# lawmurray/BayesLogit

Hardware: NVIDIA B200
Metric: pg_draws_per_sec (higher is better)
Workload: dtype f64

## Files before the change

### bayeslogit_b200/api.py

```python
import ctypes as C

import numpy as np

from . import _lib

NA = float("nan")


def set_seed(seed):
    _lib.lib().bl_set_seed(int(seed) & 0xFFFFFFFFFFFFFFFF)


def set_device(device):
    _lib.check(_lib.lib().bl_set_device(int(device)))


def _recycle(a, num, dtype):
    a = np.asarray(a, dtype=dtype).ravel()
    if a.size != num:
        a = np.resize(a, num)
    return np.ascontiguousarray(a)


def _ptr(a):
# ... 70 lines not shown


_SEEDED = {"devroye": ("bl_rpg_devroye_seeded", np.int32), "gamma": ("bl_rpg_gamma_seeded", np.float64),
           "alt": ("bl_rpg_alt_seeded", np.float64), "sp": ("bl_rpg_sp_seeded", np.float64),
           "hybrid": ("bl_rpg_hybrid_seeded", np.float64)}
_TAPE = {k: v[0].replace("_seeded", "_tape") for k, v in _SEEDED.items()}
_TAPE["devroye_plain"] = "bl_rpg_devroye_plain_tape"


def rpg_seeded(method, shape, z, seed, call_id=0, obs0=0, trunc=200):
    fn, dt = _SEEDED[method]
    z = np.ascontiguousarray(z, dtype=np.float64)
    shape = np.ascontiguousarray(shape, dtype=dt)
    num = z.size
    x = np.zeros(num)
    args = [_ptr(x), _ptr(shape), _ptr(z), num]
    it = None
    if method == "gamma":
        args.append(int(trunc))
    if method == "sp":
        it = np.zeros(num, dtype=np.int32)
        args.append(_ptr(it))
    st = getattr(_lib.lib(), fn)(*args, int(seed), int(call_id), int(obs0))
    _lib.check(st)
    return (x, it) if method == "sp" else x


def rpg_tape(method, shape, z, tape, trunc=200, trace=True):
    fn = _TAPE[method]
    dt = np.int32 if method.startswith("devroye") else np.float64
    z = np.ascontiguousarray(z, dtype=np.float64)
    shape = np.ascontiguousarray(shape, dtype=dt)
    num = z.size
    x = np.zeros(num)
    t = _lib.Tape()
    keep = []
    for k in "ueng":
        a = tape.get(k)
        if a is None:
            setattr(t, "t" + k, None)
            setattr(t, "l" + k, 0)
        else:
            a = np.ascontiguousarray(a, dtype=np.float64)
            assert a.ndim == 2 and a.shape[0] == num
            keep.append(a)
            setattr(t, "t" + k, a.ctypes.data)
            setattr(t, "l" + k, a.shape[1])
    tr = np.zeros((num, _lib.TRACE_W), dtype=np.int32) if trace else None
    args = [_ptr(x), _ptr(shape), _ptr(z), num]
    it = None
    if method == "gamma":
        args.append(int(trunc))
    if method == "sp":
        it = np.zeros(num, dtype=np.int32)
        args.append(_ptr(it))
    st = getattr(_lib.lib(), fn)(*args, C.byref(t), _ptr(tr) if trace else None)
    _lib.check(st)
    out = [x]
    if trace:
        out.append(tr)
    if it is not None:
        out.append(it)
    return tuple(out) if len(out) > 1 else x


def pg_moments(b, z):
    b = np.ascontiguousarray(b, dtype=np.float64)
    z = np.ascontiguousarray(z, dtype=np.float64)
    m1, m2 = np.zeros(b.size), np.zeros(b.size)
    _lib.check(_lib.lib().bl_probe_pg_moments(_ptr(m1), _ptr(m2), _ptr(b), _ptr(z), b.size))
    return m1, m2


def v_eval(y):
    y = np.ascontiguousarray(y, dtype=np.float64)
    v = np.zeros(y.size)
    _lib.check(_lib.lib().bl_probe_v_eval(_ptr(v), _ptr(y), y.size))
    return v


SPECFUN = {"p_norm": 0, "log_p_norm": 1, "p_gamma_rate": 2, "p_igauss": 3, "lgamma": 4, "tgamma": 5,
           "dev_right_mass": 6, "dev_coef": 7, "upper_gamma_cf": 8, "p_igauss_direct": 9, "sp_log_cos_rt": 10,
           "sp_v_table": 11, "sp_pl": 12, "sp_pl_estimate": 13,
           "alt_pr": 14, "alt_pr_estimate": 15}


def specfun(which, a, b=None, c=None):
    a = np.ascontiguousarray(a, dtype=np.float64)
    b = a if b is None else np.ascontiguousarray(np.broadcast_to(b, a.shape), dtype=np.float64)
    c = a if c is None else np.ascontiguousarray(np.broadcast_to(c, a.shape), dtype=np.float64)
    out = np.zeros(a.size)
    _lib.check(_lib.lib().bl_probe_specfun(_ptr(out), SPECFUN[which], _ptr(a), _ptr(b), _ptr(c), a.size))
    return out


def philox4x32_10(ctr, key):
    ctr = np.ascontiguousarray(ctr, dtype=np.uint32)
    key = np.ascontiguousarray(key, dtype=np.uint32)
    out = np.zeros(4, dtype=np.uint32)
    _lib.check(_lib.lib().bl_probe_philox(_ptr(out), _ptr(ctr), _ptr(key)))
    return out
```

### bayeslogit_b200/csrc/pg_alt.cuh

```cuda
#pragma once

namespace bl {

template <class Src>
__device__ __forceinline__ double alt_rtinvchi2(Src &s, double h, double trunc)
{
    double h2 = h * h;
    double R = trunc / h2;
    double E1 = s.expon();
    double E2 = s.expon();
    while ((E1 * E1) > (2 * E2 / R)) {
        E1 = s.expon();
        E2 = s.expon();
    }
    double X = 1 + E1 * R;
    X = R / (X * X);
    return h2 * X;
}

__device__ __forceinline__ double alt_pigauss(double x, double z, double lambda)
{
    double sq = sqrt(lambda / x);
    double b = sq * (x * z - 1);
    double a = sq * (x * z + 1) * -1.0;
    return p_norm(b) + ool::exp_(2 * lambda * z) * p_norm(a);
}

enum AltField {
    kAltH = 0,
    kAltTrunc,
    kAltPr,
    kAltCoef,
    kAltLgh,
    kAltLd0, kAltLd1,
    kAltLtB, kAltLtC0, kAltLtLM,
    kAltPrBand,
    kAltSetupDoubles
};
constexpr int kAltStateDoubles = 2 * kAltSetupDoubles;

struct AltState {
    double f[kAltStateDoubles];
    __device__ __forceinline__ double get(int k) const { return f[k]; }
};

struct AltStateRef {
    const double *o;
    size_t stride;
    __device__ __forceinline__ double get(int k) const { return o[(size_t)k * stride]; }
};

__device__ __forceinline__ void alt_plan(double h, int &nfull, int &nrem, double &hrem)
{
    double n = floor((h - 1.0) / 4.0);
    double remain = h - 4.0 * n;
    nfull = (int)n;
    if (remain > 4.0) {
        nrem = 2;
        hrem = 0.5 * remain;
    } else {
        nrem = 1;
        hrem = remain;
    }
}

static __device__ __noinline__ double alt_pr_fp64(double h, double z, double trunc)
{
    const double kLog2 = 0.693147180559945309417232;
    double wl, wr;
    if (z != 0)
        wl = ool::exp_(h * (kLog2 - z)) * alt_pigauss(trunc, z / h, h * h);
    else
        wl = ool::exp_(h * kLog2) * (1.0 - p_gamma_rate(1 / trunc, 0.5, 0.5 * h * h));
    double lambda_z = kPi * kPi * 0.125 + 0.5 * z * z;
    wr = ool::exp_(h * ool::log_((0.5 * kPi) / lambda_z)) * (1.0 - p_gamma_rate(trunc, h, lambda_z));
    return wr / (wr + wl);
}

constexpr double kAltPrBandWidth = 2e-5;

__device__ __forceinline__ float alt_pr_estimate(double h, double z, double trunc)
{
    const float hf = (float)h, zf = (float)z, tf = (float)trunc;
    if (!(zf < 12.0f)) return -1.0f;
    const float s = hf * rsqrtf(tf);
    const float tz = tf * zf / hf;
    const float b = s * (tz - 1.0f), na = s * (tz + 1.0f);
    const float phib = 0.5f * erfcf(-b * 0.70710678f);
    const float wl = exp2f(hf) * (__expf(-hf * zf) * phib
                                  + 0.5f * erfcxf(na * 0.70710678f) * __expf(hf * zf - 0.5f * na * na));
    const float lam = 1.2337005501361697f + 0.5f * zf * zf;
    const float x = tf * lam;
    const float lpre = hf * __logf(x) - x;
    float Q;
    if (x < hf + 1.0f) {
        float term = 1.0f, sum = 1.0f, ap = hf;
        for (int k = 0; k < 60; ++k) {
            ap += 1.0f;
            term *= x / ap;
            sum += term;
            if (term < 1e-8f * sum) break;
        }
        Q = 1.0f - sum * __expf(lpre - lgammaf(hf + 1.0f));
    } else {
        float cf = upper_gamma_cf_f32(hf, x);
        if (!(cf > 0.0f)) return -1.0f;
        Q = cf * __expf(lpre - lgammaf(hf));
    }
    if (!(Q > 0.0f)) return -1.0f;
    const float wr = __expf(hf * __logf(1.5707963267948966f / lam)) * Q;
    const float pr = wr / (wr + wl);
    return pr >= 0.0f && pr <= 1.0f ? pr : -1.0f;
}

template <bool kEstimatePr>
static __device__ __noinline__ void alt_setup(double h, double z, double *out)
{
    const double kLog2 = 0.693147180559945309417232;
    int idx = (int)floor((h - 1.0) * 100.0);
    double trunc = PG_TRUNC_SCHEDULE[idx];
    double rate_z = 0.125 * kPi * kPi + 0.5 * z * z;
    float est = kEstimatePr ? alt_pr_estimate(h, z, trunc) : -1.0f;
    out[kAltH] = h;
    out[kAltTrunc] = trunc;
    out[kAltPr] = est >= 0.0f ? (double)est : alt_pr_fp64(h, z, trunc);
    out[kAltPrBand] = est >= 0.0f ? kAltPrBandWidth : 0.0;
    out[kAltCoef] = ool::exp_(h * kLog2 - 0.5 * 1.8378770664093454835606594728112 );
    out[kAltLgh] = ool::lgamma_(h);
    out[kAltLd0] = ool::log_(h);
    out[kAltLd1] = ool::log_(2.0 + h);
    double b = rate_z * trunc;
    double d1 = b - h;
    double d3 = h - 1.0;
    double c0 = 0.5 * (d1 + sqrt(d1 * d1 + 4.0 * b)) / b;
    out[kAltLtB] = b;
    out[kAltLtC0] = c0;
    out[kAltLtLM] = d3 * ool::log_(d3 / (1.0 - c0)) - d3;
}

template <class St>
__device__ __forceinline__ bool alt_pick_right(double u, const St &st, int o, double z)
{
    const double pr = st.get(o + kAltPr), band = st.get(o + kAltPrBand);
    if (u < pr - band) return true;
    if (u > pr + band || band == 0.0) return false;
    return u < alt_pr_fp64(st.get(o + kAltH), z, st.get(o + kAltTrunc));
}

struct AltLane {
    double X, alpha, sum;
    int trial;
    int phase;
    int nfull;
    int nrem;
    __device__ __forceinline__ void start(int nf, int nr)
    {
        X = 0.0; alpha = 0.0; sum = 0.0; trial = 0; phase = 0; nfull = nf; nrem = nr;
    }
};

__device__ __forceinline__ double alt_coef(double n, double lx3, double ldn, double x, double h,
                                           double coef_h, double &g)
{
    double d_n = 2.0 * n + h;
    if (n != 0)
        g *= (n + h - 1) / n;
    else
        g = 1.0;
    double coef = coef_h * g;
    double log_kernel = -0.5 * (lx3 + d_n * d_n / x) + ldn;
    return coef * ool::exp_(log_kernel);
}

template <class Src, class St>
__device__ __forceinline__ bool alt_pick(Src &src, AltLane &L, double z, const St &st)
{
    const int o = L.nfull > 0 ? 0 : kAltSetupDoubles;
    if (L.trial >= 10000) {
        L.sum += -1.0;
        L.trial = 0;
        if (L.nfull > 0)
            L.nfull--;
        else
            L.nrem--;
        return L.nfull == 0 && L.nrem == 0;
    }
    L.trial++;
    if (alt_pick_right(src.unif(), st, o, z)) {
        L.phase = 1;
    } else {
        L.phase = (st.get(o + kAltH) / z > st.get(o + kAltTrunc)) ? 2 : 3;
        L.alpha = 0.0;
    }
    return false;
}

template <class St>
static __device__ __noinline__ bool alt_series_exact(double X, double u, double h, double trunc, const St &st, int o)
{
    const int max_inner = 200;
    const double coef_h = st.get(o + kAltCoef);
    const double lx3 = ool::log_(X * X * X);
    double g = 1.0;
    double S = alt_coef(0.0, lx3, st.get(o + kAltLd0), X, h, coef_h, g);
    double a_n = S;
    double gt;
    if (X > trunc)
        gt = ool::exp_(h * 0.45158270528945486472619522989488  + (h - 1) * (lx3 * (1.0 / 3.0))
                       - kPi * kPi * 0.125 * X - st.get(o + kAltLgh));
    else
        gt = h * ool::exp_(h * 0.693147180559945309417232 - 0.5 * (1.8378770664093454835606594728112 + lx3)
                           - 0.5 * h * h / X);
    double Y = u * gt;
    int n = 0;
    bool go = true, accept = false;
    while (go && n < max_inner) {
        ++n;
        double prev = a_n;
        double ldn = n == 1 ? st.get(o + kAltLd1) : ool::log_(2.0 * n + h);
        a_n = alt_coef((double)n, lx3, ldn, X, h, coef_h, g);
// ... 123 lines not shown
```

### bayeslogit_b200/csrc/pg_hybrid.cu

```cuda
#include <algorithm>
#include <cstdlib>
#include <vector>

#include "engine.h"
#include "pg_devroye_fast.cuh"
#include "pg_stream.cuh"

namespace bl {

namespace {

constexpr int kBinThreads = 256;
constexpr int kMetaCounts = 0;
constexpr int kMetaOffsets = 8;
constexpr int kMetaCursor = 16;

__global__ void __launch_bounds__(kBinThreads)
k_hyb_count(const double *__restrict__ h, int n, int *__restrict__ meta)
{
    __shared__ int cnt[8];
    if (threadIdx.x < 8) cnt[threadIdx.x] = 0;
    __syncthreads();
    int local[6] = {0, 0, 0, 0, 0, 0};
    for (int i = blockIdx.x * blockDim.x + threadIdx.x; i < n; i += gridDim.x * blockDim.x)
// ... 27 lines not shown
    constexpr int kCells = kBinPer * (kBinThreads / 32);
    __shared__ int wcnt[kCells][8];
    __shared__ int base[8];
    const int lane = threadIdx.x & 31, warp = threadIdx.x >> 5;
    const unsigned lt = (1u << lane) - 1u;
    const int tile_obs = kBinThreads * kBinPer;
    int tiles = (n + tile_obs - 1) / tile_obs;
    for (int tile = blockIdx.x; tile < tiles; tile += gridDim.x) {
        int reg[kBinPer], rank[kBinPer];
#pragma unroll
        for (int k = 0; k < kBinPer; ++k) {
            int i = tile * tile_obs + k * kBinThreads + threadIdx.x;
            reg[k] = i < n ? regime_of(h[i]) : -1;
        }
#pragma unroll
        for (int k = 0; k < kBinPer; ++k) {
            int i = tile * tile_obs + k * kBinThreads + threadIdx.x;
            if (reg[k] == kRegZero) x[i] = 0.0;
            rank[k] = 0;
#pragma unroll
            for (int r = 1; r < 6; ++r) {
                unsigned m = __ballot_sync(0xffffffffu, reg[k] == r);
                if (reg[k] == r) rank[k] = __popc(m & lt);
                if (lane == 0) wcnt[k * (kBinThreads / 32) + warp][r] = __popc(m);
            }
        }
        __syncthreads();
        if (threadIdx.x >= 1 && threadIdx.x < 6) {
            int r = threadIdx.x, run = 0;
            for (int c = 0; c < kCells; ++c) {
                int v = wcnt[c][r];
                wcnt[c][r] = run;
                run += v;
            }
            base[r] = run ? meta[kMetaOffsets + r] + atomicAdd(&meta[kMetaCursor + r], run) : 0;
        }
        __syncthreads();
#pragma unroll
        for (int k = 0; k < kBinPer; ++k) {
            if (reg[k] > 0) {
                int i = tile * tile_obs + k * kBinThreads + threadIdx.x;
                idx[base[reg[k]] + wcnt[k * (kBinThreads / 32) + warp][reg[k]] + rank[k]] = i;
            }
        }
        __syncthreads();
    }
}

template <int R, bool kChains = false>
__global__ void __launch_bounds__(128)
k_hyb_regime(double *__restrict__ x, const double *__restrict__ h, const double *__restrict__ z,
             const int *__restrict__ idx, const int *__restrict__ meta, StreamId id)
{
    const int count = meta[kMetaCounts + R];
    const int *list = idx + meta[kMetaOffsets + R];
    for (int j = blockIdx.x * blockDim.x + threadIdx.x; j < count; j += gridDim.x * blockDim.x) {
        int i = list[j];
        PhiloxSource s;
        if (kChains) open_batch_stream(s, id, i);
        else s.open(id.seed, id.obs0 + (uint64_t)i, id.call_id);
        double b = h[i], zi = z[i], v;
        if (R == kRegNormal) {
            double m = pg_m1(b, zi);
            double var = pg_m2(b, zi) - m * m;
            v = m + sqrt(var) * s.norm();
        } else if (R == kRegSP) {
            sp_draw(s, v, b, zi);
        } else if (R == kRegDevroye) {
            v = devroye_sum_fast(s, (int)b, zi);
        } else if (R == kRegAlt) {
            v = alt_draw(s, b, zi);
        } else {
            v = gamma_sum(s, b, zi, 200);
        }
        x[i] = v;
    }
}

__global__ void __launch_bounds__(128, 8)
k_sp_setup(const double *__restrict__ h, const double *__restrict__ z, const int *__restrict__ idx,
           const int *__restrict__ meta, double *__restrict__ state, int c0, int cap)
{
    const int count = min(meta[kMetaCounts + kRegSP] - c0, cap);
    const int *list = idx + meta[kMetaOffsets + kRegSP] + c0;
    for (int j = blockIdx.x * blockDim.x + threadIdx.x; j < count; j += gridDim.x * blockDim.x) {
        int i = list[j];
        SpState s;
        sp_setup<true>(h[i], z[i], s);
#pragma unroll
        for (int k = 0; k < kSpStateDoubles; ++k) state[(size_t)k * cap + j] = s.f[k];
    }
}

constexpr int kLaneChunk = 128;

constexpr int kRgThreads = 256;

template <int F, int D, int I>
struct RgSlots {
    double f[F][kRgThreads];
    double d[D][kRgThreads];
    uint4 buf[kRgThreads];
    uint32_t blk[kRgThreads];
    int pos[kRgThreads];
    int i[I][kRgThreads];
    int obs[kRgThreads];
    int phase[kRgThreads];
    int perm[kRgThreads];
    int wcnt[kRgThreads / 32][3];
};

struct SpRegroup {
    static constexpr int F = kSpStateDoubles, D = 3, I = 1, kClasses = 2, kRegime = kRegSP;
    using Slots = RgSlots<F, D, I>;
    __device__ static void begin(Slots &S, int t, double shape, double zraw, PhiloxSource &src)
    {
        S.d[0][t] = shape;
        S.d[1][t] = 0.5 * fabs(zraw);
        S.d[2][t] = 2.0;
        S.i[0][t] = 1;
        SpStateRef st{&S.f[0][t], (size_t)kRgThreads};
        S.phase[t] = sp_pick_left(src.unif(), st, shape) ? 1 : 2;
    }
    __device__ static bool advance(Slots &S, int sl, PhiloxSource &src, double &omega)
    {
        SpLane L;
        L.X = S.d[2][sl];
        L.iter = S.i[0][sl];
        L.phase = S.phase[sl];
        const double n = S.d[0][sl];
        SpStateRef st{&S.f[0][sl], (size_t)kRgThreads};
        bool done = sp_trip_staged(src, L, n, S.d[1][sl], st);
        if (!done && L.phase == 0) {
            if (L.iter >= 200) {
                done = true;
            } else {
                L.iter++;
                L.phase = sp_pick_left(src.unif(), st, n) ? 1 : 2;
            }
        }
        if (done) {
            omega = n * 0.25 * L.X;
        } else {
            S.d[2][sl] = L.X;
            S.i[0][sl] = L.iter;
            S.phase[sl] = L.phase;
        }
        return done;
    }
};

struct AltRegroup {
    static constexpr int F = kAltStateDoubles, D = 4, I = 3, kClasses = 3, kRegime = kRegAlt;
    using Slots = RgSlots<F, D, I>;
    __device__ static void load(const Slots &S, int sl, AltLane &L)
    {
        L.X = S.d[1][sl]; L.alpha = S.d[2][sl]; L.sum = S.d[3][sl];
        L.trial = S.i[0][sl]; L.nfull = S.i[1][sl]; L.nrem = S.i[2][sl];
        L.phase = S.phase[sl];
    }
    __device__ static void store(Slots &S, int sl, const AltLane &L)
    {
        S.d[1][sl] = L.X; S.d[2][sl] = L.alpha; S.d[3][sl] = L.sum;
        S.i[0][sl] = L.trial; S.i[1][sl] = L.nfull; S.i[2][sl] = L.nrem;
        S.phase[sl] = L.phase;
    }
    __device__ static void begin(Slots &S, int t, double shape, double zraw, PhiloxSource &src)
    {
        int nfull, nrem;
        double hrem;
        alt_plan(shape, nfull, nrem, hrem);
        AltLane L;
        L.start(nfull, nrem);
// ... 332 lines not shown
```

### bayeslogit_b200/csrc/pg_kernels.cu

```cuda
#include "engine.h"
#include "pg_devroye_fast.cuh"
#include "pg_stream.cuh"

namespace bl {

namespace {

constexpr int kThreads = 128;

inline int grid_for(int64_t num, int threads, int ctas_per_sm)
{
    int64_t need = (num + threads - 1) / threads;
    int64_t cap = 148LL * ctas_per_sm;
    return (int)(need < cap ? (need > 0 ? need : 1) : cap);
}

template <int M, class Src>
__device__ __forceinline__ double draw_one(Src &s, const void *shape, const double *z, int64_t i,
                                           int trunc, int *iter, int &aux)
{
    aux = 0;
    if (M == kDevroye || M == kDevroyeLoop) {
        int n = ((const int *)shape)[i];
        return n != 0 ? devroye_sum_fast(s, n, z[i]) : 0.0;
// ... 11 lines not shown
        if (h != 0) {
            double d;
            aux = sp_draw(s, d, h, z[i]);
            if (iter) iter[i] = aux;
            return d;
        }
        return 0.0;
    } else {
        double h = ((const double *)shape)[i];
        return hybrid_draw(s, h, z[i], aux);
    }
}

template <int M, bool kChains = false>
__global__ void __launch_bounds__(kThreads)
k_rpg_philox(double *__restrict__ x, const void *__restrict__ shape, const double *__restrict__ z,
             int64_t num, int trunc, int *__restrict__ iter, StreamId id)
{
    int64_t stride = (int64_t)gridDim.x * blockDim.x;
    for (int64_t i = (int64_t)blockIdx.x * blockDim.x + threadIdx.x; i < num; i += stride) {
        PhiloxSource s;
        if (kChains) open_batch_stream(s, id, i);
        else s.open(id.seed, id.obs0 + (uint64_t)i, id.call_id);
        int aux;
        x[i] = draw_one<M>(s, shape, z, i, trunc, iter, aux);
    }
}

template <int M>
__global__ void __launch_bounds__(kThreads)
k_rpg_tape(double *__restrict__ x, const void *__restrict__ shape, const double *__restrict__ z,
           int64_t num, int trunc, int *__restrict__ iter, DevTape tp, int *__restrict__ trace)
{
    int64_t stride = (int64_t)gridDim.x * blockDim.x;
    for (int64_t i = (int64_t)blockIdx.x * blockDim.x + threadIdx.x; i < num; i += stride) {
        TapeSource s;
        s.open(tp.tu, tp.lu, tp.te, tp.le, tp.tn, tp.ln, tp.tg, tp.lg, (size_t)i);
        int aux;
        double v = draw_one<M>(s, shape, z, i, trunc, iter, aux);
        x[i] = s.exhausted() ? nan("") : v;
        if (trace) {
            int *t = trace + i * BL_TRACE_W;
            s.counts(t);
            t[4] = s.exhausted() ? 1 : 0;
            t[5] = aux;
        }
    }
}

__global__ void k_probe_moments(double *m1, double *m2, const double *b, const double *z, int64_t num)
{
    int64_t i = (int64_t)blockIdx.x * blockDim.x + threadIdx.x;
    if (i < num) {
        m1[i] = pg_m1(b[i], z[i]);
        m2[i] = pg_m2(b[i], z[i]);
    }
}

__global__ void k_probe_v_eval(double *v, const double *y, int64_t num)
{
    int64_t i = (int64_t)blockIdx.x * blockDim.x + threadIdx.x;
    if (i < num) v[i] = v_eval(y[i]);
}

__global__ void k_probe_specfun(double *out, int which, const double *a, const double *b,
                                const double *c, int64_t num)
{
    int64_t i = (int64_t)blockIdx.x * blockDim.x + threadIdx.x;
    if (i >= num) return;
    double r = 0.0;
    switch (which) {
    case 0: r = p_norm(a[i]); break;
    case 1: r = log_p_norm(a[i]); break;
    case 2: r = p_gamma_rate(a[i], b[i], c[i]); break;
    case 3: r = p_igauss(a[i], b[i], c[i]); break;
    case 4: r = lgamma(a[i]); break;
    case 5: r = tgamma(a[i]); break;
    case 6: r = dev_right_mass(a[i]); break;
    case 7: r = dev_coef((int)b[i], a[i]); break;
    case 8: r = upper_gamma_cf(b[i], a[i]); break;
    case 9: r = p_igauss_direct(a[i], b[i], c[i]); break;
    case 10: { double v, g; sp_vg(a[i], v, g); r = g; break; }
    case 11: { double v, g; r = sp_vg_table(a[i], v, g) ? v : nan(""); break; }
    case 12: { SpState st; sp_setup<false>(a[i], b[i], st); r = st.f[kSpPl]; break; }
    case 13: { SpState st; sp_setup<true>(a[i], b[i], st); r = st.f[kSpPlBand] > 0.0 ? st.f[kSpPl] : nan(""); break; }
    case 14: { double f[kAltSetupDoubles]; alt_setup<false>(a[i], 0.5 * fabs(b[i]), f); r = f[kAltPr]; break; }
    case 15: { double f[kAltSetupDoubles]; alt_setup<true>(a[i], 0.5 * fabs(b[i]), f); r = f[kAltPrBand] > 0.0 ? f[kAltPr] : nan(""); break; }
    }
    out[i] = r;
}

__global__ void k_probe_philox(uint32_t *out4, const uint32_t *ctr4, const uint32_t *key2)
{
    uint4 r = Philox4x32::block(make_uint4(ctr4[0], ctr4[1], ctr4[2], ctr4[3]),
                                make_uint2(key2[0], key2[1]));
    out4[0] = r.x; out4[1] = r.y; out4[2] = r.z; out4[3] = r.w;
}

template <int M, bool kChains = false>
cudaError_t launch_philox_m(double *x, const void *shape, const double *z, int64_t num, int trunc,
                            int *iter, StreamId id, cudaStream_t st)
{
    if (num <= 0) return cudaSuccess;
    k_rpg_philox<M, kChains><<<grid_for(num, kThreads, 16), kThreads, 0, st>>>(x, shape, z, num, trunc, iter, id);
    count_launch();
    return cudaGetLastError();
}

template <int M>
cudaError_t launch_tape_m(double *x, const void *shape, const double *z, int64_t num, int trunc,
                          int *iter, DevTape tp, int *trace, cudaStream_t st)
{
    if (num <= 0) return cudaSuccess;
    k_rpg_tape<M><<<grid_for(num, kThreads, 16), kThreads, 0, st>>>(x, shape, z, num, trunc, iter, tp, trace);
    count_launch();
    return cudaGetLastError();
}

}

cudaError_t launch_rpg(Method m, double *x, const void *shape, const double *z, int64_t num,
                       int trunc, int *iter, StreamId id, cudaStream_t st)
{
    switch (m) {
    case kDevroye: return launch_devroye_refill(x, (const int *)shape, z, num, id, st);
    case kDevroyeLoop: return launch_philox_m<kDevroyeLoop>(x, shape, z, num, trunc, iter, id, st);
    case kGamma: return launch_philox_m<kGamma>(x, shape, z, num, trunc, iter, id, st);
    case kAlt: return launch_philox_m<kAlt>(x, shape, z, num, trunc, iter, id, st);
    case kSP: return launch_philox_m<kSP>(x, shape, z, num, trunc, iter, id, st);
    case kHybrid:
        return id.chain_len ? launch_philox_m<kHybrid, true>(x, shape, z, num, trunc, iter, id, st)
                            : launch_philox_m<kHybrid>(x, shape, z, num, trunc, iter, id, st);
    case kDevroyePlain: return launch_philox_m<kDevroyePlain>(x, shape, z, num, trunc, iter, id, st);
    }
    return cudaErrorInvalidValue;
}

cudaError_t launch_rpg_tape(Method m, double *x, const void *shape, const double *z, int64_t num,
                            int trunc, int *iter, DevTape tp, int *trace, cudaStream_t st)
{
    switch (m) {
    case kDevroye: return launch_tape_m<kDevroye>(x, shape, z, num, trunc, iter, tp, trace, st);
    case kGamma: return launch_tape_m<kGamma>(x, shape, z, num, trunc, iter, tp, trace, st);
    case kAlt: return launch_tape_m<kAlt>(x, shape, z, num, trunc, iter, tp, trace, st);
    case kSP: return launch_tape_m<kSP>(x, shape, z, num, trunc, iter, tp, trace, st);
    case kHybrid: return launch_tape_m<kHybrid>(x, shape, z, num, trunc, iter, tp, trace, st);
    case kDevroyePlain: return launch_tape_m<kDevroyePlain>(x, shape, z, num, trunc, iter, tp, trace, st);
    case kDevroyeLoop: return launch_tape_m<kDevroye>(x, shape, z, num, trunc, iter, tp, trace, st);
    }
    return cudaErrorInvalidValue;
}

cudaError_t launch_probe_moments(double *m1, double *m2, const double *b, const double *z,
                                 int64_t num, cudaStream_t st)
{
    if (num <= 0) return cudaSuccess;
    k_probe_moments<<<(unsigned)((num + 127) / 128), 128, 0, st>>>(m1, m2, b, z, num);
    count_launch();
    return cudaGetLastError();
}

cudaError_t launch_probe_v_eval(double *v, const double *y, int64_t num, cudaStream_t st)
{
    if (num <= 0) return cudaSuccess;
    k_probe_v_eval<<<(unsigned)((num + 127) / 128), 128, 0, st>>>(v, y, num);
    count_launch();
    return cudaGetLastError();
}

cudaError_t launch_probe_specfun(double *out, int which, const double *a, const double *b,
// ... 18 lines not shown
```

### bayeslogit_b200/csrc/pg_sp.cuh

```cuda
#pragma once

#include "pg_sp_tables.h"

namespace bl {

__device__ __forceinline__ double y_of_v(double v, double tol)
{
    double r = sqrt(fabs(v));
    if (v > tol) return ool::tan_(r) / r;
    if (v < -1 * tol) return ool::tanh_(r) / r;
    return 1.0;
}

static __device__ __noinline__ double v_eval_ref(double y)
{
    const double tol = 1e-9;
    const int max_iter = 1000;
    if (y < PG_YGRID[0]) return -1. / (y * y);
    if (y > PG_YGRID[PG_YGRID_LEN - 1]) {
        double v = ool::atan_(0.5 * y * kPi);
        return v * v;
    }
    if (y == 1) return 0.0;
    double id = (ool::log_(y) / ool::log_(2.0) + 4.0) / 0.1;
    int idlow = (int)id;
    int idhigh = idlow + 1;
    if (idhigh > PG_VGRID_LEN - 1) idhigh = PG_VGRID_LEN - 1;
    double vl = PG_VGRID[idlow];
    double vh = PG_VGRID[idhigh];
    int iter = 0;
    double diff = tol + 1.0;
    double vnew = vl, vold = vl;
    while (diff > tol && iter < max_iter) {
        iter++;
        vold = vnew;
        double yv = y_of_v(vold, 1e-8);
        double f0 = yv - y;
        double f1;
        if (fabs(vold) >= 1e-8)
            f1 = 0.5 * (yv * yv + (1 - yv) / vold);
        else
            f1 = 0.5 * (yv * yv);
        vnew = vold - f0 / f1;
        vnew = vnew > vh ? vh : vnew;
        vnew = vnew < vl ? vl : vnew;
        diff = fabs(vnew - vold);
    }
    return vnew;
}

__device__ __forceinline__ double sp_cos_rt(double v)
{
    double r = sqrt(fabs(v));
    return v >= 0 ? ool::cos_(r) : ool::cosh_(r);
}

__device__ __forceinline__ bool sp_vg_table(double y, double &v, double &g)
{
    if (!(y >= 0.0625 && y < 16.0)) return false;
    if (fabs(y - 1.0) < 1e-6) return false;
    float tt = (__log2f((float)y) + 4.0f) * 10.0f;
    float fr = tt - floorf(tt);
    float margin = tt > 48.0f ? 2e-4f : 5e-5f;
    if (fr < margin || fr > 1.0f - margin) return false;
    int hi = __double2hiint(y), lo = __double2loint(y);
    int e = (hi >> 20) - 1023;
    int j = (hi >> (20 - SP_TAB_K)) & ((1 << SP_TAB_K) - 1);
    double f = __hiloint2double((hi & 0x000FFFFF) | 0x3FF00000, lo);
    double u = (f - 1.0) * (double)(2 << SP_TAB_K) - (double)(2 * j + 1);
    int row = ((e - SP_TAB_ELO) << SP_TAB_K) + j;
    const double2 *cv = reinterpret_cast<const double2 *>(SP_VTAB + row * (SP_TAB_DEG + 1));
    const double2 *cg = reinterpret_cast<const double2 *>(SP_GTAB + row * (SP_TAB_DEG + 1));
    double2 a = __ldg(cv), b = __ldg(cg);
    double pv = fma(a.x, u, a.y), pg = fma(b.x, u, b.y);
#pragma unroll
    for (int k = 1; k < (SP_TAB_DEG + 1) / 2; ++k) {
        a = __ldg(cv + k);
        b = __ldg(cg + k);
        pv = fma(fma(pv, u, a.x), u, a.y);
        pg = fma(fma(pg, u, b.x), u, b.y);
    }
    v = pv;
    g = pg;
    return true;
}

static __device__ __noinline__ void sp_vg_ref(double y, double &v, double &g)
{
    v = v_eval_ref(y);
    g = ool::log_(sp_cos_rt(v));
}

__device__ __forceinline__ void sp_vg(double y, double &v, double &g)
{
    if (!sp_vg_table(y, v, g)) sp_vg_ref(y, v, g);
}

__device__ __forceinline__ double v_eval(double y)
{
    double v, g;
    if (sp_vg_table(y, v, g)) return v;
    return v_eval_ref(y);
}

enum SpField {
    kSpMd = 0,
    kSpPl,
    kSpRt2rl,
    kSpRl, kSpIl,
    kSpRr, kSpIr,
    kSpCl, kSpCr,
    kSpLmd,
    kSpLcz,
    kSpLcn,
    kSpLtB, kSpLtC0, kSpLtLM,
    kSpLLtB,
    kSpMu,
    kSpC1md,
    kSpPlBand,
    kSpStateDoubles
};

struct SpState {
    double f[kSpStateDoubles];
    __device__ __forceinline__ double get(int k) const { return f[k]; }
};

struct SpStateRef {
    const double *o;
    size_t stride;
    __device__ __forceinline__ double get(int k) const { return o[(size_t)k * stride]; }
};

__device__ __forceinline__ void sp_tangent(double x, double z, double mid, double lcz, bool right,
                                           double &slope, double &icept)
{
    double v, g;
    sp_vg(x, v, g);
    double u = 0.5 * v;
    double t = u + 0.5 * z * z;
    double phi_val = lcz - g - t * x;
    double phi_der = -1.0 * t;
    double delta_val, delta_der;
    if (right) {
        delta_val = 0.087011376989629699;
        delta_der = 1.0 / x;
    } else {
        delta_val = 0.5 * (1 - 1.0 / x) - 0.5 * (1 - 1.0 / mid);
        delta_der = 0.5 / (x * x);
    }
    double eta_val = phi_val - delta_val;
    double eta_der = phi_der - delta_der;
    slope = eta_der;
    icept = eta_val - eta_der * x;
}

static __device__ __noinline__ double sp_wr_ref(double hra, double lcn, double n, double rr, double ir,
                                                double lmd, double md)
{
    return ool::exp_(hra + lcn - n * ool::log_(n * rr) + n * ir - n * lmd) * ool::tgamma_(n)
         * (1.0 - p_gamma_rate(md, n, n * rr));
}

__device__ __forceinline__ bool sp_cf_form_applies(double n, double ltb)
{
    double dx = ltb - n;
    return dx >= 1.0 && n <= 171.0 && dx * dx <= 12.0 * (ltb + n);
}

__device__ __forceinline__ double sp_pl_fp64(double n, double md, double rt2rl, double il, double ir, double rr,
                                             double hla, double hra, double lmd, double lcn, double ltb)
{
    double wl = ool::exp_(hla - n * rt2rl + n * il + 0.5 * n * 1. / md) * p_igauss_direct(md, 1. / rt2rl, n);
    double wr;
    if (sp_cf_form_applies(n, ltb))
        wr = ool::exp_(hra + lcn + n * ir - ltb) * upper_gamma_cf(n, ltb);
    else
        wr = sp_wr_ref(hra, lcn, n, rr, ir, lmd, md);
    return wl / (wl + wr);
}

constexpr double kSpPlBandWidth = 2e-5;

__device__ __forceinline__ float sp_pl_estimate(double n, double md, double rt2rl, double il, double ir,
                                                double lmd, double lcn, double ltb)
{
    if (!sp_cf_form_applies(n, ltb)) return -1.0f;
    const double D = -0.5 * lmd + lcn + n * (ir - il) - ltb + n * rt2rl - 0.5 * n / md;
    if (!(fabs(D) < 60.0)) return -1.0f;
    const float s = sqrtf((float)(n / md));
    const float b = s * (float)(md * rt2rl - 1.0);
    const float t = s * (float)(md * rt2rl + 1.0) * 0.70710678f;
    const float pig = 0.5f * erfcf(-b * 0.70710678f) + 0.5f * erfcxf(t) * __expf(-0.5f * b * b);
    const float hcf = upper_gamma_cf_f32((float)n, (float)ltb);
    if (!(hcf > 0.0f) || !(pig > 0.0f)) return -1.0f;
    const float R = __expf((float)D) * hcf / pig;
    if (!(R >= 0.0f) || isinf(R)) return -1.0f;
    return 1.0f / (1.0f + R);
}

template <class St>
static __device__ __noinline__ double sp_pl_from_state(const St &s, double n)
{
    double lcn = s.get(kSpLcn);
    return sp_pl_fp64(n, s.get(kSpMd), s.get(kSpRt2rl), s.get(kSpIl), s.get(kSpIr), s.get(kSpRr),
                      s.get(kSpCl) - lcn, s.get(kSpCr) - lcn, s.get(kSpLmd), lcn, s.get(kSpLtB));
}

template <class St>
__device__ __forceinline__ bool sp_pick_left(double u, const St &s, double n)
{
    const double pl = s.get(kSpPl), band = s.get(kSpPlBand);
    if (u < pl - band) return true;
    if (u > pl + band || band == 0.0) return false;
    return u < sp_pl_from_state(s, n);
}

template <bool kEstimatePl = false>
__device__ __forceinline__ void sp_setup(double n, double zraw, SpState &s)
{
    double z = 0.5 * fabs(zraw);
    double xl = y_of_v(-1 * z * z, 1e-6);
    double md = xl * 1.1;
    double xr = xl * 1.2;
    double vmd = v_eval(md);
    double K2md;
    if (fabs(vmd) >= 1e-6)
        K2md = md * md + (1 - md) / vmd;
    else
        K2md = md * md;
    double m2 = md * md;
    double al = m2 * md / K2md;
    double ar = m2 / K2md;
    double lcz;
    if (kEstimatePl) {
        float zf = (float)z;
        lcz = zf < 12.0f ? (double)__logf(coshf(zf)) : (double)(zf - 0.69314718f);
    } else {
        lcz = ool::log_(ool::cosh_(z));
    }
    double sl, il, sr, ir;
    sp_tangent(xl, z, md, lcz, false, sl, il);
    sp_tangent(xr, z, md, lcz, true, sr, ir);
    double rl = -1. * sl;
    double rr = -1. * sr;
    double lcn = 0.5 * ool::log_(0.5 * n / kPi);
    double rt2rl = sqrt(2 * rl);
    double lmd = ool::log_(md);
    double hla = 0.5 * ool::log_(al), hra = hla - 0.5 * lmd;
    (void)ar;
    double ltb = (n * rr) * md;
    double pl, pl_band = 0.0;
    float est = kEstimatePl ? sp_pl_estimate(n, md, rt2rl, il, ir, lmd, lcn, ltb) : -1.0f;
    if (est >= 0.0f) {
        pl = (double)est;
        pl_band = kSpPlBandWidth;
    } else {
        pl = sp_pl_fp64(n, md, rt2rl, il, ir, rr, hla, hra, lmd, lcn, ltb);
    }
    double d1 = ltb - n;
    double d3 = n - 1.0;
    double c0 = 0.5 * (d1 + sqrt(d1 * d1 + 4.0 * ltb)) / ltb;
    double l_M = d3 * ool::log_(d3 / (1.0 - c0)) - d3;
    s.f[kSpMd] = md;
    s.f[kSpPl] = pl;
    s.f[kSpPlBand] = pl_band;
    s.f[kSpRt2rl] = rt2rl;
    s.f[kSpRl] = rl;
    s.f[kSpIl] = il;
    s.f[kSpRr] = rr;
    s.f[kSpIr] = ir;
    s.f[kSpCl] = hla + lcn;
    s.f[kSpCr] = hra + lcn;
    s.f[kSpLmd] = lmd;
    s.f[kSpLcz] = lcz;
    s.f[kSpLcn] = lcn;
    s.f[kSpLtB] = ltb;
    s.f[kSpLtC0] = c0;
    s.f[kSpLtLM] = l_M;
    s.f[kSpLLtB] = ool::log_(ltb);
    s.f[kSpMu] = 1. / rt2rl;
    s.f[kSpC1md] = 1. - 1. / md;
}

template <class St>
__device__ __forceinline__ double sp_density(double x, double n, double z, const St &s)
{
    double v, g;
    sp_vg(x, v, g);
    double u = 0.5 * v;
    double z2 = z * z;
    double t = u + 0.5 * z2;
    double phi = s.get(kSpLcz) - g - t * x;
    double K2;
    if (fabs(v) >= 1e-6)
        K2 = x * x + (1 - x) / v;
    else
        K2 = x * x;
    double log_spa = s.get(kSpLcn) - 0.5 * ool::log_(K2) + n * phi;
    return ool::exp_(log_spa);
}

struct SpLane {
    double X;
    int iter;
    int phase;
    __device__ __forceinline__ void start() { X = 2.0; iter = 0; phase = 0; }
};

template <class Src, class St>
__device__ __forceinline__ bool sp_trip(Src &src, SpLane &L, double n, double z, const St &s)
{
    const int maxiter = 200;
    const double md = s.get(kSpMd);
    if (L.phase == 0) {
        if (L.iter >= maxiter) return true;
        L.iter++;
        L.phase = sp_pick_left(src.unif(), s, n) ? 1 : 2;
    }
    if (L.phase == 1) {
        double mu = 1. / s.get(kSpRt2rl);
        if (md < mu) {
            double X = md + 1.0, alpha = 0.0;
            while (src.unif() > alpha) {
                X = rtinvchi2(src, n, md);
                alpha = ool::exp_(-0.5 * n / (mu * mu) * X);
            }
            L.X = X;
            L.phase = 3;
        } else {
            double X = igauss(src, mu, n);
            if (!(X > md)) {
                L.X = X;
                L.phase = 3;
            }
        }
    } else if (L.phase == 2) {
        if (n > 1.0 && md > 0.0) {
            double b = s.get(kSpLtB), c0 = s.get(kSpLtC0);
            double x = b + src.expon() / c0;
            double u = src.unif();
            double l_rho = (n - 1.0) * ool::log_(x) - x * (1.0 - c0);
            if (ool::log_(u) <= l_rho - s.get(kSpLtLM)) {
                L.X = md * (x / b);
                L.phase = 4;
            }
        } else {
            L.X = ltgamma(src, n, n * s.get(kSpRr), md);
            L.phase = 4;
        }
    }
    if (L.phase >= 3) {
        double X = L.X, F;
        if (L.phase == 3) {
            double phi_ev = n * (s.get(kSpIl) - s.get(kSpRl) * X) + 0.5 * n * ((1. - 1. / X) - (1. - 1. / md));
            F = ool::exp_(s.get(kSpCl) - 1.5 * ool::log_(X) + phi_ev);
        } else {
            double phi_ev = n * (s.get(kSpIr) - s.get(kSpRr) * X) + n * (ool::log_(X) - s.get(kSpLmd));
            F = ool::exp_(s.get(kSpCr) + phi_ev) / X;
        }
        double spa = sp_density(X, n, z, s);
        if (F * src.unif() < spa) return true;
        L.phase = 0;
        if (L.iter >= maxiter) return true;
    }
// ... 138 lines not shown
```

### bayeslogit_b200/csrc/specfun.cuh

```cuda
#pragma once

#include <cmath>

namespace bl {

constexpr double kPi = 3.141592653589793238462643383279502884197;
constexpr double kSqrt1_2 = 0.70710678118654752440;

__device__ __forceinline__ double p_norm(double x) { return 0.5 * erfc(-x * kSqrt1_2); }

static __device__ __noinline__ double log_p_norm(double x)
{
    if (x > 0.0) return log1p(-0.5 * erfc(x * kSqrt1_2));
    double t = -x * kSqrt1_2;
    return log(0.5 * erfcx(t)) - t * t;
}

__device__ inline double gamma_log_prefix(double a, double x)
{
    if (a < 10.0) return a * log(x) - x - lgamma(a);
    double mu = (x - a) / a;
    double phi = mu - log1p(mu);
    double ia = 1.0 / a, ia2 = ia * ia;
    double S = ia * (1.0 / 12 - ia2 * (1.0 / 360 - ia2 * (1.0 / 1260 - ia2 * (1.0 / 1680
             - ia2 * (1.0 / 1188 - ia2 * (691.0 / 360360 - ia2 * (1.0 / 156)))))));
    return -a * phi - S + 0.5 * log(a / (2.0 * 3.14159265358979323846));
}

static __device__ __noinline__ double p_gamma_lower(double a, double x)
{
    if (x <= 0.0) return 0.0;
    if (isinf(x)) return 1.0;
    double lpre = gamma_log_prefix(a, x);
    if (x < a + 1.0) {
        double ap = a, del = 1.0 / a, sum = del;
        for (int n = 0; n < 2000; ++n) {
            ap += 1.0;
            del *= x / ap;
            sum += del;
            if (fabs(del) < fabs(sum) * 1e-17) break;
        }
        return sum * exp(lpre);
    }
    const double tiny = 1e-300;
    double b = x + 1.0 - a;
    double c = 1.0 / tiny;
    double d = 1.0 / b;
    double h = d;
    for (int i = 1; i < 2000; ++i) {
        double an = -(double)i * ((double)i - a);
        b += 2.0;
        d = an * d + b;
        if (fabs(d) < tiny) d = tiny;
        c = b + an / c;
        if (fabs(c) < tiny) c = tiny;
        d = 1.0 / d;
        double del = d * c;
        h *= del;
        if (fabs(del - 1.0) < 1e-16) break;
    }
    return 1.0 - exp(lpre) * h;
}

__device__ __forceinline__ double upper_gamma_cf(double a, double x)
{
    double b = x + 1.0 - a;
    double A0 = 0.0, B0 = 1.0;
    double A1 = 1.0, B1 = b;
    double det = 1.0, di = 0.0;
    for (int i = 1; i < 2000; ++i) {
        di += 1.0;
        double an = -di * (di - a);
        b += 2.0;
        double A2 = fma(b, A1, an * A0);
        double B2 = fma(b, B1, an * B0);
        det *= -an;
        A0 = A1; B0 = B1; A1 = A2; B1 = B2;
        if (fabs(det) <= 1e-16 * fabs(A1 * B0)) break;
        if (fabs(B1) > 0x1p200) {
            A0 *= 0x1p-200; B0 *= 0x1p-200; A1 *= 0x1p-200; B1 *= 0x1p-200;
            det *= 0x1p-400;
        }
    }
    return A1 / B1;
}

__device__ __forceinline__ float upper_gamma_cf_f32(float a, float x)
{
    float bb = x + 1.0f - a;
    float c = 1e30f, d = 1.0f / bb, h = d;
    for (int i = 1; i <= 64; ++i) {
        float an = -(float)i * ((float)i - a);
        bb += 2.0f;
        d = an * d + bb;
        d = fabsf(d) < 1e-30f ? 1e-30f : d;
        c = bb + an / c;
        c = fabsf(c) < 1e-30f ? 1e-30f : c;
        d = 1.0f / d;
        float del = d * c;
        h *= del;
        if (fabsf(del - 1.0f) < 3e-7f) return h;
    }
    return -1.0f;
}

__device__ __forceinline__ double p_igauss_direct(double x, double mu, double lambda)
{
    double Z = 1.0 / mu;
    double s = sqrt(lambda / x);
    double b = s * (x * Z - 1.0);
    double t = s * (x * Z + 1.0) * kSqrt1_2;
    return 0.5 * erfc(-b * kSqrt1_2) + 0.5 * erfcx(t) * exp(2.0 * lambda * Z - t * t);
}

__device__ __forceinline__ double p_gamma_rate(double x, double shape, double rate)
{
    return p_gamma_lower(shape, x * rate);
}

__device__ __forceinline__ double p_igauss(double x, double mu, double lambda)
{
    double Z = 1.0 / mu;
    double s = sqrt(lambda / x);
    double b = s * (x * Z - 1.0);
    double a = -1.0 * s * (x * Z + 1.0);
    return exp(log_p_norm(b)) + exp(2.0 * lambda * Z + log_p_norm(a));
}

}
```

Measured before the change: 5.081 billion.

## Streamline SP and alt setup with table lookups, shape-4 constants, division-free CF

```diff
diff --git a/bayeslogit_b200/api.py b/bayeslogit_b200/api.py
--- a/bayeslogit_b200/api.py
+++ b/bayeslogit_b200/api.py
@@ -176,7 +176,8 @@
 SPECFUN = {"p_norm": 0, "log_p_norm": 1, "p_gamma_rate": 2, "p_igauss": 3, "lgamma": 4, "tgamma": 5,
            "dev_right_mass": 6, "dev_coef": 7, "upper_gamma_cf": 8, "p_igauss_direct": 9, "sp_log_cos_rt": 10,
            "sp_v_table": 11, "sp_pl": 12, "sp_pl_estimate": 13,
-           "alt_pr": 14, "alt_pr_estimate": 15}
+           "alt_pr": 14, "alt_pr_estimate": 15, "sp_setup_field": 16, "sp_setup_field_binned": 17,
+           "alt_setup_field": 18, "alt_setup_field_binned": 19}
 
 
 def specfun(which, a, b=None, c=None):
diff --git a/bayeslogit_b200/csrc/pg_alt.cuh b/bayeslogit_b200/csrc/pg_alt.cuh
--- a/bayeslogit_b200/csrc/pg_alt.cuh
+++ b/bayeslogit_b200/csrc/pg_alt.cuh
@@ -79,21 +79,22 @@
 
 constexpr double kAltPrBandWidth = 2e-5;
 
+template <bool kShape4 = false>
 __device__ __forceinline__ float alt_pr_estimate(double h, double z, double trunc)
 {
-    const float hf = (float)h, zf = (float)z, tf = (float)trunc;
+    const float hf = kShape4 ? 4.0f : (float)h, zf = (float)z, tf = (float)trunc;
     if (!(zf < 12.0f)) return -1.0f;
-    const float s = hf * rsqrtf(tf);
+    const float s = kShape4 ? 1.9682714f  : hf * rsqrtf(tf);
     const float tz = tf * zf / hf;
     const float b = s * (tz - 1.0f), na = s * (tz + 1.0f);
     const float phib = 0.5f * erfcf(-b * 0.70710678f);
-    const float wl = exp2f(hf) * (__expf(-hf * zf) * phib
+    const float wl = (kShape4 ? 16.0f : exp2f(hf)) * (__expf(-hf * zf) * phib
                                   + 0.5f * erfcxf(na * 0.70710678f) * __expf(hf * zf - 0.5f * na * na));
     const float lam = 1.2337005501361697f + 0.5f * zf * zf;
     const float x = tf * lam;
     const float lpre = hf * __logf(x) - x;
     float Q;
-    if (x < hf + 1.0f) {
+    if (!kShape4 && x < hf + 1.0f) {
         float term = 1.0f, sum = 1.0f, ap = hf;
         for (int k = 0; k < 60; ++k) {
             ap += 1.0f;
@@ -105,7 +106,7 @@
     } else {
         float cf = upper_gamma_cf_f32(hf, x);
         if (!(cf > 0.0f)) return -1.0f;
-        Q = cf * __expf(lpre - lgammaf(hf));
+        Q = cf * __expf(lpre - (kShape4 ? 1.7917595f  : lgammaf(hf)));
     }
     if (!(Q > 0.0f)) return -1.0f;
     const float wr = __expf(hf * __logf(1.5707963267948966f / lam)) * Q;
@@ -113,13 +114,38 @@
     return pr >= 0.0f && pr <= 1.0f ? pr : -1.0f;
 }
 
+__device__ __forceinline__ void alt_ltgamma_consts(double h, double rate_z, double trunc, double *out)
+{
+    double b = rate_z * trunc;
+    double d1 = b - h;
+    double d3 = h - 1.0;
+    double c0 = 0.5 * (d1 + sqrt(d1 * d1 + 4.0 * b)) / b;
+    out[kAltLtB] = b;
+    out[kAltLtC0] = c0;
+    out[kAltLtLM] = d3 * ool::log_(d3 / (1.0 - c0)) - d3;
+}
+
 template <bool kEstimatePr>
 static __device__ __noinline__ void alt_setup(double h, double z, double *out)
 {
     const double kLog2 = 0.693147180559945309417232;
+    double rate_z = 0.125 * kPi * kPi + 0.5 * z * z;
+    if (kEstimatePr && h == 4.0) {
+        const double trunc = PG_TRUNC_SCHEDULE[PG_TRUNC_SCHEDULE_LEN - 1];
+        const float est = alt_pr_estimate<true>(4.0, z, trunc);
+        out[kAltH] = 4.0;
+        out[kAltTrunc] = trunc;
+        out[kAltPr] = est >= 0.0f ? (double)est : alt_pr_fp64(4.0, z, trunc);
+        out[kAltPrBand] = est >= 0.0f ? kAltPrBandWidth : 0.0;
+        out[kAltCoef] = 0x1.9884533d43650p+2;
+        out[kAltLgh] = 0x1.cab0bfa2a2002p+0;
+        out[kAltLd0] = 0x1.62e42fefa39efp+0;
+        out[kAltLd1] = 0x1.cab0bfa2a2002p+0;
+        alt_ltgamma_consts(4.0, rate_z, trunc, out);
+        return;
+    }
     int idx = (int)floor((h - 1.0) * 100.0);
     double trunc = PG_TRUNC_SCHEDULE[idx];
-    double rate_z = 0.125 * kPi * kPi + 0.5 * z * z;
     float est = kEstimatePr ? alt_pr_estimate(h, z, trunc) : -1.0f;
     out[kAltH] = h;
     out[kAltTrunc] = trunc;
@@ -129,13 +155,7 @@
     out[kAltLgh] = ool::lgamma_(h);
     out[kAltLd0] = ool::log_(h);
     out[kAltLd1] = ool::log_(2.0 + h);
-    double b = rate_z * trunc;
-    double d1 = b - h;
-    double d3 = h - 1.0;
-    double c0 = 0.5 * (d1 + sqrt(d1 * d1 + 4.0 * b)) / b;
-    out[kAltLtB] = b;
-    out[kAltLtC0] = c0;
-    out[kAltLtLM] = d3 * ool::log_(d3 / (1.0 - c0)) - d3;
+    alt_ltgamma_consts(h, rate_z, trunc, out);
 }
 
 template <class St>
diff --git a/bayeslogit_b200/csrc/pg_hybrid.cu b/bayeslogit_b200/csrc/pg_hybrid.cu
--- a/bayeslogit_b200/csrc/pg_hybrid.cu
+++ b/bayeslogit_b200/csrc/pg_hybrid.cu
@@ -133,13 +133,10 @@
            const int *__restrict__ meta, double *__restrict__ state, int c0, int cap)
 {
     const int count = min(meta[kMetaCounts + kRegSP] - c0, cap);
-    const int *list = idx + meta[kMetaOffsets + kRegSP] + c0;
+    const int first = meta[kMetaOffsets + kRegSP] + c0;
     for (int j = blockIdx.x * blockDim.x + threadIdx.x; j < count; j += gridDim.x * blockDim.x) {
-        int i = list[j];
-        SpState s;
-        sp_setup<true>(h[i], z[i], s);
-#pragma unroll
-        for (int k = 0; k < kSpStateDoubles; ++k) state[(size_t)k * cap + j] = s.f[k];
+        int i = idx[first + j];
+        sp_setup_binned(h[i], z[i], state + j, (size_t)cap);
     }
 }
 
diff --git a/bayeslogit_b200/csrc/pg_kernels.cu b/bayeslogit_b200/csrc/pg_kernels.cu
--- a/bayeslogit_b200/csrc/pg_kernels.cu
+++ b/bayeslogit_b200/csrc/pg_kernels.cu
@@ -117,10 +117,14 @@
     case 9: r = p_igauss_direct(a[i], b[i], c[i]); break;
     case 10: { double v, g; sp_vg(a[i], v, g); r = g; break; }
     case 11: { double v, g; r = sp_vg_table(a[i], v, g) ? v : nan(""); break; }
-    case 12: { SpState st; sp_setup<false>(a[i], b[i], st); r = st.f[kSpPl]; break; }
-    case 13: { SpState st; sp_setup<true>(a[i], b[i], st); r = st.f[kSpPlBand] > 0.0 ? st.f[kSpPl] : nan(""); break; }
+    case 12: { SpState st; sp_setup(a[i], b[i], st); r = st.f[kSpPl]; break; }
+    case 13: { SpState st; sp_setup_binned(a[i], b[i], st.f, 1); r = st.f[kSpPlBand] > 0.0 ? st.f[kSpPl] : nan(""); break; }
     case 14: { double f[kAltSetupDoubles]; alt_setup<false>(a[i], 0.5 * fabs(b[i]), f); r = f[kAltPr]; break; }
     case 15: { double f[kAltSetupDoubles]; alt_setup<true>(a[i], 0.5 * fabs(b[i]), f); r = f[kAltPrBand] > 0.0 ? f[kAltPr] : nan(""); break; }
+    case 16: { SpState st; sp_setup(a[i], b[i], st); r = st.f[(int)c[i]]; break; }
+    case 17: { SpState st; sp_setup_binned(a[i], b[i], st.f, 1); r = st.f[(int)c[i]]; break; }
+    case 18: { double f[kAltSetupDoubles]; alt_setup<false>(a[i], 0.5 * fabs(b[i]), f); r = f[(int)c[i]]; break; }
+    case 19: { double f[kAltSetupDoubles]; alt_setup<true>(a[i], 0.5 * fabs(b[i]), f); r = f[(int)c[i]]; break; }
     }
     out[i] = r;
 }
diff --git a/bayeslogit_b200/csrc/pg_sp.cuh b/bayeslogit_b200/csrc/pg_sp.cuh
--- a/bayeslogit_b200/csrc/pg_sp.cuh
+++ b/bayeslogit_b200/csrc/pg_sp.cuh
@@ -55,8 +55,10 @@
     return v >= 0 ? ool::cos_(r) : ool::cosh_(r);
 }
 
-__device__ __forceinline__ bool sp_vg_table(double y, double &v, double &g)
-{
+__device__ __forceinline__ bool sp_tab_locate(double y, int &row, double &u)
+{
+    row = 0;
+    u = 0.0;
     if (!(y >= 0.0625 && y < 16.0)) return false;
     if (fabs(y - 1.0) < 1e-6) return false;
     float tt = (__log2f((float)y) + 4.0f) * 10.0f;
@@ -67,8 +69,29 @@
     int e = (hi >> 20) - 1023;
     int j = (hi >> (20 - SP_TAB_K)) & ((1 << SP_TAB_K) - 1);
     double f = __hiloint2double((hi & 0x000FFFFF) | 0x3FF00000, lo);
-    double u = (f - 1.0) * (double)(2 << SP_TAB_K) - (double)(2 * j + 1);
-    int row = ((e - SP_TAB_ELO) << SP_TAB_K) + j;
+    u = (f - 1.0) * (double)(2 << SP_TAB_K) - (double)(2 * j + 1);
+    row = ((e - SP_TAB_ELO) << SP_TAB_K) + j;
+    return true;
+}
+
+__device__ __forceinline__ double sp_tab_eval(const double *tab, int row, double u)
+{
+    const double2 *c = reinterpret_cast<const double2 *>(tab + row * (SP_TAB_DEG + 1));
+    double2 a = __ldg(c);
+    double p = fma(a.x, u, a.y);
+#pragma unroll
+    for (int k = 1; k < (SP_TAB_DEG + 1) / 2; ++k) {
+        a = __ldg(c + k);
+        p = fma(fma(p, u, a.x), u, a.y);
+    }
+    return p;
+}
+
+__device__ __forceinline__ bool sp_vg_table(double y, double &v, double &g)
+{
+    int row;
+    double u;
+    if (!sp_tab_locate(y, row, u)) return false;
     const double2 *cv = reinterpret_cast<const double2 *>(SP_VTAB + row * (SP_TAB_DEG + 1));
     const double2 *cg = reinterpret_cast<const double2 *>(SP_GTAB + row * (SP_TAB_DEG + 1));
     double2 a = __ldg(cv), b = __ldg(cg);
@@ -132,13 +155,16 @@
     __device__ __forceinline__ double get(int k) const { return o[(size_t)k * stride]; }
 };
 
-__device__ __forceinline__ void sp_tangent(double x, double z, double mid, double lcz, bool right,
-                                           double &slope, double &icept)
-{
-    double v, g;
-    sp_vg(x, v, g);
-    double u = 0.5 * v;
-    double t = u + 0.5 * z * z;
+__device__ __forceinline__ double sp_ltgamma_c0(double b, double n)
+{
+    const double d1 = __dsub_rn(b, n);
+    return 0.5 * (d1 + sqrt(fma(4.0, b, d1 * d1))) / b;
+}
+
+__device__ __forceinline__ void sp_tangent_vg(double x, double v, double g, double z, double mid, double lcz,
+                                              bool right, double &slope, double &icept)
+{
+    double t = fma(0.5, v, 0.5 * z * z);
     double phi_val = lcz - g - t * x;
     double phi_der = -1.0 * t;
     double delta_val, delta_der;
@@ -153,6 +179,14 @@
     double eta_der = phi_der - delta_der;
     slope = eta_der;
     icept = eta_val - eta_der * x;
+}
+
+__device__ __forceinline__ void sp_tangent(double x, double z, double mid, double lcz, bool right,
+                                           double &slope, double &icept)
+{
+    double v, g;
+    sp_vg(x, v, g);
+    sp_tangent_vg(x, v, g, z, mid, lcz, right, slope, icept);
 }
 
 static __device__ __noinline__ double sp_wr_ref(double hra, double lcn, double n, double rr, double ir,
@@ -182,13 +216,13 @@
 
 constexpr double kSpPlBandWidth = 2e-5;
 
-__device__ __forceinline__ float sp_pl_estimate(double n, double md, double rt2rl, double il, double ir,
-                                                double lmd, double lcn, double ltb)
+__device__ __forceinline__ float sp_pl_estimate(double n, double md, double rmd, double rt2rl, double il,
+                                                double ir, double lmd, double lcn, double ltb)
 {
     if (!sp_cf_form_applies(n, ltb)) return -1.0f;
-    const double D = -0.5 * lmd + lcn + n * (ir - il) - ltb + n * rt2rl - 0.5 * n / md;
+    const double D = -0.5 * lmd + lcn + n * (ir - il) - ltb + n * rt2rl - 0.5 * n * rmd;
     if (!(fabs(D) < 60.0)) return -1.0f;
-    const float s = sqrtf((float)(n / md));
+    const float s = sqrtf((float)(n * rmd));
     const float b = s * (float)(md * rt2rl - 1.0);
     const float t = s * (float)(md * rt2rl + 1.0) * 0.70710678f;
     const float pig = 0.5f * erfcf(-b * 0.70710678f) + 0.5f * erfcxf(t) * __expf(-0.5f * b * b);
@@ -216,7 +250,6 @@
     return u < sp_pl_from_state(s, n);
 }
 
-template <bool kEstimatePl = false>
 __device__ __forceinline__ void sp_setup(double n, double zraw, SpState &s)
 {
     double z = 0.5 * fabs(zraw);
@@ -231,14 +264,7 @@
         K2md = md * md;
     double m2 = md * md;
     double al = m2 * md / K2md;
-    double ar = m2 / K2md;
-    double lcz;
-    if (kEstimatePl) {
-        float zf = (float)z;
-        lcz = zf < 12.0f ? (double)__logf(coshf(zf)) : (double)(zf - 0.69314718f);
-    } else {
-        lcz = ool::log_(ool::cosh_(z));
-    }
+    double lcz = ool::log_(ool::cosh_(z));
     double sl, il, sr, ir;
     sp_tangent(xl, z, md, lcz, false, sl, il);
     sp_tangent(xr, z, md, lcz, true, sr, ir);
@@ -248,23 +274,14 @@
     double rt2rl = sqrt(2 * rl);
     double lmd = ool::log_(md);
     double hla = 0.5 * ool::log_(al), hra = hla - 0.5 * lmd;
-    (void)ar;
     double ltb = (n * rr) * md;
-    double pl, pl_band = 0.0;
-    float est = kEstimatePl ? sp_pl_estimate(n, md, rt2rl, il, ir, lmd, lcn, ltb) : -1.0f;
-    if (est >= 0.0f) {
-        pl = (double)est;
-        pl_band = kSpPlBandWidth;
-    } else {
-        pl = sp_pl_fp64(n, md, rt2rl, il, ir, rr, hla, hra, lmd, lcn, ltb);
-    }
-    double d1 = ltb - n;
+    double pl = sp_pl_fp64(n, md, rt2rl, il, ir, rr, hla, hra, lmd, lcn, ltb);
     double d3 = n - 1.0;
-    double c0 = 0.5 * (d1 + sqrt(d1 * d1 + 4.0 * ltb)) / ltb;
+    double c0 = sp_ltgamma_c0(ltb, n);
     double l_M = d3 * ool::log_(d3 / (1.0 - c0)) - d3;
     s.f[kSpMd] = md;
     s.f[kSpPl] = pl;
-    s.f[kSpPlBand] = pl_band;
+    s.f[kSpPlBand] = 0.0;
     s.f[kSpRt2rl] = rt2rl;
     s.f[kSpRl] = rl;
     s.f[kSpIl] = il;
@@ -281,6 +298,76 @@
     s.f[kSpLLtB] = ool::log_(ltb);
     s.f[kSpMu] = 1. / rt2rl;
     s.f[kSpC1md] = 1. - 1. / md;
+}
+
+__device__ __forceinline__ void sp_setup_binned(double n, double zraw, double *o, size_t stride)
+{
+    auto put = [&](int k, double v) { o[(size_t)k * stride] = v; };
+    const double z = 0.5 * fabs(zraw);
+    const double xl = y_of_v(-1 * z * z, 1e-6);
+    const double md = xl * 1.1;
+    const double xr = xl * 1.2;
+    int rowm, rowr, rowl;
+    double um, ur, ul;
+    const bool okm = sp_tab_locate(md, rowm, um);
+    const bool okr = sp_tab_locate(xr, rowr, ur);
+    const bool okl = sp_tab_locate(xl, rowl, ul);
+    double vmd = sp_tab_eval(SP_VTAB, rowm, um);
+    double vr = sp_tab_eval(SP_VTAB, rowr, ur), gr = sp_tab_eval(SP_GTAB, rowr, ur);
+    double gl = sp_tab_eval(SP_GTAB, rowl, ul);
+    if (!okm) vmd = v_eval_ref(md);
+    if (!okr) sp_vg_ref(xr, vr, gr);
+    const float zf = (float)z;
+    const double lcz = zf < 12.0f ? (double)__logf(coshf(zf)) : (double)(zf - 0.69314718f);
+    const double rmd = 1.0 / md;
+    double rl, il;
+    if (okl) {
+        rl = 0.5 / (xl * xl);
+        const double rxl = 2.0 * rl * xl;
+        il = (lcz - gl) - (0.5 * (1.0 - rxl) - 0.5 * (1.0 - rmd)) + rl * xl;
+    } else {
+        double vl, sl;
+        sp_vg_ref(xl, vl, gl);
+        sp_tangent_vg(xl, vl, gl, z, md, lcz, false, sl, il);
+        rl = -1. * sl;
+    }
+    double sr, ir;
+    sp_tangent_vg(xr, vr, gr, z, md, lcz, true, sr, ir);
+    const double rr = -1. * sr;
+    const double rt2rl = sqrt(2 * rl);
+    const double ltb = (n * rr) * md;
+    const double m2 = md * md;
+    const double al = fabs(vmd) >= 1e-6 ? m2 * md * vmd / fma(m2, vmd, 1.0 - md) : md;
+    put(kSpMd, md);
+    put(kSpRt2rl, rt2rl);
+    put(kSpMu, 1. / rt2rl);
+    put(kSpRl, rl);
+    put(kSpIl, il);
+    put(kSpRr, rr);
+    put(kSpIr, ir);
+    put(kSpLcz, lcz);
+    put(kSpLtB, ltb);
+    put(kSpC1md, 1. - rmd);
+    const double lcn = 0.5 * ool::log_(n * (0.5 / kPi));
+    const double lmd = ool::log_(md);
+    const double hla = 0.5 * ool::log_(al), hra = hla - 0.5 * lmd;
+    put(kSpLcn, lcn);
+    put(kSpLmd, lmd);
+    put(kSpCl, hla + lcn);
+    put(kSpCr, hra + lcn);
+    const float est = sp_pl_estimate(n, md, rmd, rt2rl, il, ir, lmd, lcn, ltb);
+    if (est >= 0.0f) {
+        put(kSpPl, (double)est);
+        put(kSpPlBand, kSpPlBandWidth);
+    } else {
+        put(kSpPl, sp_pl_fp64(n, md, rt2rl, il, ir, rr, hla, hra, lmd, lcn, ltb));
+        put(kSpPlBand, 0.0);
+    }
+    const double d3 = n - 1.0;
+    const double c0 = sp_ltgamma_c0(ltb, n);
+    put(kSpLtC0, c0);
+    put(kSpLtLM, d3 * ool::log_(d3 / (1.0 - c0)) - d3);
+    put(kSpLLtB, ool::log_(ltb));
 }
 
 template <class St>
diff --git a/bayeslogit_b200/csrc/specfun.cuh b/bayeslogit_b200/csrc/specfun.cuh
--- a/bayeslogit_b200/csrc/specfun.cuh
+++ b/bayeslogit_b200/csrc/specfun.cuh
@@ -87,19 +87,23 @@
 
 __device__ __forceinline__ float upper_gamma_cf_f32(float a, float x)
 {
-    float bb = x + 1.0f - a;
-    float c = 1e30f, d = 1.0f / bb, h = d;
+    float b = x + 1.0f - a;
+    float A0 = 0.0f, B0 = 1.0f;
+    float A1 = 1.0f, B1 = b;
+    float det = 1.0f, di = 0.0f;
     for (int i = 1; i <= 64; ++i) {
-        float an = -(float)i * ((float)i - a);
-        bb += 2.0f;
-        d = an * d + bb;
-        d = fabsf(d) < 1e-30f ? 1e-30f : d;
-        c = bb + an / c;
-        c = fabsf(c) < 1e-30f ? 1e-30f : c;
-        d = 1.0f / d;
-        float del = d * c;
-        h *= del;
-        if (fabsf(del - 1.0f) < 3e-7f) return h;
+        di += 1.0f;
+        const float an = -di * (di - a);
+        b += 2.0f;
+        const float A2 = fmaf(b, A1, an * A0);
+        const float B2 = fmaf(b, B1, an * B0);
+        det *= -an;
+        A0 = A1; B0 = B1; A1 = A2; B1 = B2;
+        if (fabsf(det) <= 3e-7f * fabsf(A1 * B0)) return A1 / B1;
+        if (fabsf(B1) > 0x1p40f) {
+            A0 *= 0x1p-40f; B0 *= 0x1p-40f; A1 *= 0x1p-40f; B1 *= 0x1p-40f;
+            det *= 0x1p-80f;
+        }
     }
     return -1.0f;
 }
```

New measurement: 5.274 billion (median of 6 runs). +3.8%, better.
